# Funatiq/cuclark

Measured on AMD Instinct MI355X. Metric: Mreads/sec (10M x 150bp, k=31), higher is better.
Workload: dtype u64

## Files before the change

cuclark_amd/csrc/mic_engine.hip:

```cpp
#include "mi_clark.h"
#include "mic_internal.h"

#include <errno.h>
#include <stdarg.h>
#include <stdio.h>
#include <stdlib.h>
#include <string.h>
#include <time.h>

#include <sched.h>

#include <algorithm>
#include <mutex>
#include <string>
#include <atomic>
#include <thread>
#include <unistd.h>
#include <utility>
#include <vector>

static thread_local char g_err[512] = "";
thread_local uint64_t mic_build_reserved_hbm = 0;

namespace {
// ... 48 lines not shown
  if (!out) return MIC_E_INVALID;
  StreamPool& P = pool();
  std::lock_guard<std::mutex> lk(P.mu);
  out[0] = (uint32_t)P.all_streams.size(); out[1] = (uint32_t)P.free_streams.size();
  out[2] = (uint32_t)P.all_events.size(); out[3] = (uint32_t)P.free_events.size();
  return MIC_OK;
}

void mic_event_put(hipEvent_t ev) {
  if (!ev) return;
  (void)hipEventSynchronize(ev);
  StreamPool& P = pool();
  std::lock_guard<std::mutex> lk(P.mu);
  for (const auto& a : P.all_events) if (a.second == ev) { P.free_events.push_back(a); return; }
}
namespace {
std::mutex g_report_mu;
std::string g_report;
thread_local std::string t_report;

struct Batch {
  uint32_t* h_rp = nullptr; uint16_t* h_cont = nullptr;
  uint32_t* d_rp = nullptr; uint16_t* d_cont = nullptr;
  uint32_t* d_results = nullptr; uint32_t* d_rows = nullptr;
  uint32_t* d_flagged = nullptr; uint32_t* h_flagged = nullptr;
  uint32_t* d_peer = nullptr; uint32_t* d_acc = nullptr;
  uint32_t* d_crowd = nullptr;
  size_t first_read = 0, n_reads = 0, n_cont = 0, max_reads = 0, max_cont = 0;
  hipStream_t stream = nullptr;
  hipEvent_t done = nullptr, ev_up = nullptr, ev_k = nullptr;
  bool scheduled = false, resolved = true, extended = false;
};

}

struct mic_engine {
  mic_config cfg;
  int device = 0, n_cu = 256;
  hipStream_t stream = nullptr;
  hipStream_t up_stream = nullptr, down_stream = nullptr;
  bool db_loaded = false;
  uint4* slots = nullptr;
  uint4* side = nullptr;
  uint8_t* d_sizes = nullptr;
  MicTable table;
  int slot_class = 32;
  mic_db_info info;
  std::vector<Batch> batches;
  void* h_block = nullptr; void* d_block = nullptr;
  uint32_t* h_results = nullptr; uint32_t* h_rows = nullptr;
  size_t num_reads_total = 0;
  std::mutex submit_mu;
  uint32_t* d_flagged = nullptr; uint32_t flagged_cap = 0;
  uint32_t* d_crowd = nullptr; size_t crowd_reads = 0;
  hipEvent_t ev0 = nullptr, ev1 = nullptr;
  bool timed = false;
  size_t last_n_reads = 0;
  void* ingest = nullptr;
  uint32_t min_quality = 0;
  uint32_t low_complexity = 0;
  uint64_t reserve_hbm = 0;
  uint32_t part = 0, n_parts = 0;
  MicAbund abund;
  MicRollup rollup;
  MicDensity density;
  MicSplit split;
  MicKsketch ksketch;
  MicHitmap hitmap;
};

namespace {

const uint32_t kFlaggedCap = 1u << 16;

int set_device(const mic_engine* e) {
  MIC_TRY(hipSetDevice(e->device));
  return MIC_OK;
}

void fill_table(mic_engine* e, const MicBuildOut& b, uint64_t htsize, uint64_t s0, uint64_t s1, int key_bytes,
                uint32_t sampling, int layout, int m) {
  e->slots = b.slots;
  const bool parted = (layout == MIC_LAYOUT_SUPER || layout == MIC_LAYOUT_SUPER2) && (b.part_lo != 0 || b.part_hi != b.n_main);
  e->table.slots = parted ? b.slots - (ptrdiff_t)b.part_lo * 8 : b.slots;
  e->table.slot_lo = parted ? (uint32_t)b.part_lo : 0; e->table.slot_cnt = parted ? (uint32_t)(b.part_hi - b.part_lo) : 0;
  e->table.parted = parted ? 1 : 0;
  e->side = b.side;
  e->table.side = b.side; e->table.side_mask = b.side ? (uint32_t)(b.side_cells - 1) : 0;
  e->table.n_main = b.n_main;
  e->table.shard_start = s0;
  e->table.shard_end = s1;
  e->table.div = mic_make_div(htsize);
  e->table.k = e->cfg.k;
  e->table.layout = layout == MIC_LAYOUT_MINIMIZER ? 1 : (layout == MIC_LAYOUT_SUPER || layout == MIC_LAYOUT_SUPER2) ? 2 : 0;
  e->table.fwd = layout == MIC_LAYOUT_SUPER2 ? 1 : 0;
  e->table.m = m;
  e->table.sharded = (s0 != 0 || s1 != htsize) ? 1 : 0;
  e->table.sizes = e->d_sizes;
  mic_db_info& i = e->info;
  i.htsize = htsize; i.shard_start = s0; i.shard_end = s1;
  i.n_elems = b.n_elems; i.n_elems_file = b.n_elems_file;
  const uint64_t n_res = parted ? b.part_hi - b.part_lo : b.n_main;
  i.n_slots = n_res + b.n_overflow; i.n_overflow = b.n_overflow;
  i.part = e->n_parts > 1 ? e->part : 0; i.n_parts = e->n_parts > 1 ? e->n_parts : 0;
  i.part_slot_lo = parted ? b.part_lo : 0; i.part_slot_hi = parted ? b.part_hi : 0; i.n_slots_whole = b.n_main;
  i.side_kmers = b.side ? b.side_kmers : 0; i.side_bytes = b.side ? b.side_cells * 16 : 0;
// ... 400 lines not shown
  g_peer[from][to] = ok ? 1 : -1;
  return ok;
}
void mic_peer_enable_engines(mic_engine* const* engines, size_t n) {
  for (size_t i = 0; i < n; ++i)
    for (size_t j = 0; j < n; ++j)
      if (engines[i] && engines[j] && engines[i]->device != engines[j]->device) mic_peer_enable(engines[i]->device, engines[j]->device);
}

extern "C" {

const char* mic_last_error(void) { return g_err; }

int mic_device_count(int* count) {
  int n = 0;
  hipError_t e = hipGetDeviceCount(&n);
  if (e != hipSuccess) { *count = 0; return mic_set_error(MIC_E_NODEVICE, "hipGetDeviceCount: %s", hipGetErrorString(e)); }
  *count = n;
  return MIC_OK;
}

int mic_create(const mic_config* cfg, mic_engine** out) {
  if (!cfg || !out) return mic_set_error(MIC_E_INVALID, "null argument");
  if (cfg->k < 2 || cfg->k > 32) return mic_set_error(MIC_E_INVALID, "The k-mer length should be in [2,32].");
  if (cfg->num_targets > 65535) return mic_set_error(MIC_E_INVALID, "too many targets (%u > 65535)", cfg->num_targets);
  if (cfg->layout > MIC_LAYOUT_SUPER2) return mic_set_error(MIC_E_INVALID, "unknown table layout %u", cfg->layout);
  int n = 0;
  if (hipGetDeviceCount(&n) != hipSuccess || n == 0)
    return mic_set_error(MIC_E_NODEVICE, "no HIP device available: the MI355X engine cannot run (there is no CPU fallback)");
  int dev = cfg->device;
  if (dev < 0) { if (hipGetDevice(&dev) != hipSuccess) dev = 0; }
  if (dev >= n) return mic_set_error(MIC_E_INVALID, "device %d out of range (%d devices)", dev, n);
  hipDeviceProp_t prop;
  MIC_TRY(hipSetDevice(dev));
  MIC_TRY(hipGetDeviceProperties(&prop, dev));
  if (strncmp(prop.gcnArchName, "gfx950", 6) != 0)
    return mic_set_error(MIC_E_NODEVICE, "device %d is %s; this library carries gfx950 (MI355X) code objects only", dev, prop.gcnArchName);
  mic_engine* e = new (std::nothrow) mic_engine();
  if (!e) return mic_set_error(MIC_E_NOMEM, "out of host memory");
  e->cfg = *cfg;
  if (e->cfg.num_batches == 0) e->cfg.num_batches = 1;
  if (e->cfg.row_words == 0) e->cfg.row_words = 16;
  if (e->cfg.row_words < 2) e->cfg.row_words = 2;
  e->device = dev;
  e->n_cu = prop.multiProcessorCount;
  memset(&e->info, 0, sizeof(e->info));
  memset(&e->table, 0, sizeof(e->table));
  hipError_t he = mic_stream_get(&e->stream);
  if (he == hipSuccess) he = mic_stream_get(&e->up_stream);
  if (he == hipSuccess) he = mic_stream_get(&e->down_stream);
  if (he == hipSuccess) he = mic_event_get(&e->ev0, true);
  if (he == hipSuccess) he = mic_event_get(&e->ev1, true);
  if (he == hipSuccess) he = hipMalloc(&e->d_flagged, (size_t)(kFlaggedCap + 1) * 4);
  if (he != hipSuccess) { mic_destroy(e); return mic_set_error(MIC_E_HIP, "engine setup: %s", hipGetErrorString(he)); }
  e->flagged_cap = kFlaggedCap;
  *out = e;
  return MIC_OK;
}

int mic_destroy(mic_engine* e) {
  if (!e) return MIC_OK;
  hipSetDevice(e->device);
  hipDeviceSynchronize();
  mic_ingest_free(e);
  mic_gz_release(e);
  free_batches(e);
  if (e->slots) hipFree(e->slots);
  if (e->side) hipFree(e->side);
  if (e->d_sizes) hipFree(e->d_sizes);
  if (e->d_flagged) hipFree(e->d_flagged);
  if (e->d_crowd) hipFree(e->d_crowd);
  if (e->abund.d_counts) hipFree(e->abund.d_counts);
  if (e->rollup.d_counts) hipFree(e->rollup.d_counts);
  if (e->density.d_counts) hipFree(e->density.d_counts);
  if (e->ksketch.d_regs) hipFree(e->ksketch.d_regs);
  if (e->rollup.d_block) hipFree(e->rollup.d_block);
  if (e->ev0) mic_event_put(e->ev0);
  if (e->ev1) mic_event_put(e->ev1);
  if (e->stream) mic_stream_put(e->stream);
  if (e->up_stream) mic_stream_put(e->up_stream);
  if (e->down_stream) mic_stream_put(e->down_stream);
  delete e;
  return MIC_OK;
}

int mic_db_unload(mic_engine* e) {
  if (!e) return mic_set_error(MIC_E_INVALID, "null engine");
  int rc = set_device(e);
  if (rc) return rc;
  hipDeviceSynchronize();
  if (e->slots) hipFree(e->slots);
  if (e->side) hipFree(e->side);
  if (e->d_sizes) hipFree(e->d_sizes);
  e->slots = nullptr; e->side = nullptr; e->d_sizes = nullptr; e->db_loaded = false;
  memset(&e->info, 0, sizeof(e->info));
  return MIC_OK;
}

int mic_db_get_info(const mic_engine* e, mic_db_info* info) {
  if (!e || !info) return mic_set_error(MIC_E_INVALID, "null argument");
  if (!e->db_loaded) return mic_set_error(MIC_E_STATE, "no database loaded");
  *info = e->info;
  return MIC_OK;
}

int mic_debug_fetch_slots(mic_engine* e, uint64_t first, uint64_t n, uint32_t* out) {
  if (!e || !out) return mic_set_error(MIC_E_INVALID, "null argument");
  if (!e->db_loaded) return mic_set_error(MIC_E_STATE, "no database loaded");
  if (e->table.layout != 2 || e->table.parted) return mic_set_error(MIC_E_UNSUPPORTED, "slots are fetched from a whole super-k-mer table only");
  if (first > e->info.n_slots || n > e->info.n_slots - first) return mic_set_error(MIC_E_INVALID, "slots [%llu, +%llu) of %llu",
                                                                                   (unsigned long long)first, (unsigned long long)n, (unsigned long long)e->info.n_slots);
  int rc = set_device(e);
  if (rc) return rc;
  MIC_TRY(hipDeviceSynchronize());
  if (n) MIC_TRY(hipMemcpy(out, e->table.slots + first * 8, n * 128, hipMemcpyDeviceToHost));
  return MIC_OK;
}

const char* mic_db_last_build_report(void) {
  static thread_local std::string copy;
  std::lock_guard<std::mutex> lk(g_report_mu);
  copy = g_report;
  return copy.c_str();
// ... 572 lines not shown
  free(h_sz);
  for (Dev& dv : devs) {
    hipSetDevice(dv.device);
    if (dv.d_sz) hipFree(dv.d_sz);
    if (dv.d_ky) hipFree(dv.d_ky);
    if (dv.d_lb) hipFree(dv.d_lb);
  }
  return rc;
}

int mic_batch_check(mic_engine* e, size_t batch, int* done) {
  if (!e || batch >= e->batches.size() || !done) return mic_set_error(MIC_E_INVALID, "bad argument");
  Batch& B = e->batches[batch];
  if (!B.scheduled) { *done = 0; return MIC_OK; }
  hipError_t he = hipEventQuery(B.done);
  if (he == hipSuccess) *done = 1;
  else if (he == hipErrorNotReady) *done = 0;
  else return mic_set_error(MIC_E_HIP, "hipEventQuery: %s", hipGetErrorString(he));
  return MIC_OK;
}

int mic_thread_bind_near_device(mic_engine* e, int on) {
  if (!e) return mic_set_error(MIC_E_INVALID, "null engine");
  mic_bind_thread_near_device(e->device, on);
  return MIC_OK;
}

int mic_sync(mic_engine* e) {
  if (!e) return mic_set_error(MIC_E_INVALID, "null engine");
  int rc = set_device(e);
  if (rc) return rc;
  MIC_TRY(hipDeviceSynchronize());
  return MIC_OK;
}

int mic_batches_free(mic_engine* e) {
  if (!e) return mic_set_error(MIC_E_INVALID, "null engine");
  int rc = set_device(e);
  if (rc) return rc;
  hipDeviceSynchronize();
  free_batches(e);
  return MIC_OK;
}

int mic_query_device(mic_engine* e, const uint32_t* d_rp, const uint16_t* d_cont, size_t n_reads, uint32_t* d_results,
                     uint32_t* d_rows, void* stream) {
  if (!e || !d_rp || !d_cont || !d_results) return mic_set_error(MIC_E_INVALID, "null argument");
  if (!e->db_loaded) return mic_set_error(MIC_E_STATE, "no database loaded");
  if (n_reads > 0xFFFFFFF0ull) return mic_set_error(MIC_E_INVALID, "too many reads in one call");
  if (((uintptr_t)d_cont & 3) || ((uintptr_t)d_rp & 3)) return mic_set_error(MIC_E_INVALID, "d_containers and d_reads_pointer must be 4-byte aligned");
  int rc = set_device(e);
  if (rc) return rc;
  hipStream_t s = stream ? (hipStream_t)stream : e->stream;
  MIC_TRY(hipMemsetAsync(e->d_flagged, 0, 4, s));
  MicQueryArgs a;
  a.t = e->table; a.reads_ptr = d_rp; a.cont = d_cont; a.n_reads = (uint32_t)n_reads;
  a.row_words = e->cfg.row_words; a.results = d_results; a.rows = d_rows;
  a.flagged = e->d_flagged; a.flagged_cap = e->flagged_cap;
  if (e->table.side && n_reads > e->crowd_reads) {
    MIC_TRY(hipStreamSynchronize(s));
    if (e->d_crowd) { hipFree(e->d_crowd); e->d_crowd = nullptr; e->crowd_reads = 0; }
    MIC_TRY(hipMalloc(&e->d_crowd, mic_crowd_dims(n_reads).words * 4));
    e->crowd_reads = n_reads;
  }
  mic_crowd_attach(a, e->table.side ? e->d_crowd : nullptr, e->crowd_reads);
  MIC_TRY(hipEventRecord(e->ev0, s));
  MIC_TRY(mic_launch_query(a, e->slot_class, e->n_cu, s));
  MIC_TRY(hipEventRecord(e->ev1, s));
  e->timed = true;
  e->last_n_reads = n_reads;
  return MIC_OK;
}

int mic_last_query_ms(mic_engine* e, float* ms) {
  if (!e || !ms) return mic_set_error(MIC_E_INVALID, "null argument");
  if (!e->timed) return mic_set_error(MIC_E_STATE, "no query was launched");
  MIC_TRY(hipEventSynchronize(e->ev1));
  MIC_TRY(hipEventElapsedTime(ms, e->ev0, e->ev1));
  return MIC_OK;
}

int mic_last_crowd_stats(mic_engine* e, uint32_t out[4]) {
  if (!e || !out) return mic_set_error(MIC_E_INVALID, "null argument");
  out[0] = out[1] = out[2] = out[3] = 0;
  if (!e->timed || !e->d_crowd || !e->table.side) return MIC_OK;
  int rc = set_device(e);
  if (rc) return rc;
  MIC_TRY(hipEventSynchronize(e->ev1));
  MIC_TRY(hipMemcpy(out, e->d_crowd, 16, hipMemcpyDeviceToHost));
  return MIC_OK;
}

int mic_debug_fetch_crowd(mic_engine* e, uint32_t* out, size_t words, uint32_t caps[3]) {
  if (!e || !out || !caps) return mic_set_error(MIC_E_INVALID, "null argument");
  if (!e->d_crowd || !e->timed) return mic_set_error(MIC_E_STATE, "no work area");
  int rc = set_device(e);
  if (rc) return rc;
  const MicCrowdDims d = mic_crowd_dims(e->crowd_reads);
  caps[0] = d.pend_cap; caps[1] = d.item_cap; caps[2] = d.pool_cap;
  MIC_TRY(hipEventSynchronize(e->ev1));
  MIC_TRY(hipMemcpy(out, e->d_crowd, (words < d.words ? words : d.words) * 4, hipMemcpyDeviceToHost));
  return MIC_OK;
}

int mic_resolve_flagged_device(mic_engine* e, const uint32_t* d_rp, const uint16_t* d_cont, uint32_t* d_results,
                               uint32_t* d_rows, void* stream, size_t* n_resolved) {
  if (!e || !d_rp || !d_cont || !d_results) return mic_set_error(MIC_E_INVALID, "null argument");
  int rc = set_device(e);
  if (rc) return rc;
  hipStream_t s = stream ? (hipStream_t)stream : e->stream;
  uint32_t nf = 0;
  MIC_TRY(hipMemcpyAsync(&nf, e->d_flagged, 4, hipMemcpyDeviceToHost, s));
  MIC_TRY(hipStreamSynchronize(s));
  if (n_resolved) *n_resolved = nf;
  if (!nf) return MIC_OK;
  if (nf > e->flagged_cap) {
    if (n_resolved) *n_resolved = e->last_n_reads;
    return run_dense(e, d_rp, d_cont, nullptr, e->last_n_reads, d_results, d_rows, s);
  }
  return run_dense(e, d_rp, d_cont, e->d_flagged + 1, nf, d_results, d_rows, s);
}

int mic_merge_rows_device(mic_engine* e, const uint32_t* a, const uint32_t* b, uint32_t* out, size_t n, void* stream) {
  if (!e || !a || !b || !out) return mic_set_error(MIC_E_INVALID, "null argument");
  int rc = set_device(e);
  if (rc) return rc;
  MIC_TRY(mic_launch_merge_rows(a, b, out, e->cfg.row_words, n, nullptr, stream ? (hipStream_t)stream : e->stream));
  return MIC_OK;
}

int mic_result_from_rows_device(mic_engine* e, const uint32_t* rows, uint32_t* results, size_t n, void* stream) {
  if (!e || !rows || !results) return mic_set_error(MIC_E_INVALID, "null argument");
  int rc = set_device(e);
  if (rc) return rc;
  MIC_TRY(mic_launch_result_from_rows(rows, e->cfg.row_words, results, n, stream ? (hipStream_t)stream : e->stream));
  return MIC_OK;
}

int mic_result_from_dense_device(mic_engine* e, const uint32_t* d_counts, const uint32_t* d_ids, size_t n_ids, uint32_t* d_results,
                                 uint32_t* d_rows, void* stream) {
  if (!e || !d_counts || !d_results) return mic_set_error(MIC_E_INVALID, "null argument");
  int rc = set_device(e);
  if (rc) return rc;
  MIC_TRY(mic_launch_dense_finish(d_counts, d_ids, n_ids, e->cfg.num_targets ? e->cfg.num_targets : 1, d_results, d_rows,
                                 e->cfg.row_words, stream ? (hipStream_t)stream : e->stream));
  return MIC_OK;
}

int mic_probe_stats_device(mic_engine* e, const uint32_t* d_rp, const uint16_t* d_cont, size_t n_reads, uint64_t out[4]) {
  if (!e || !d_rp || !d_cont || !out) return mic_set_error(MIC_E_INVALID, "null argument");
  if (!e->db_loaded) return mic_set_error(MIC_E_STATE, "no database loaded");
  int rc = set_device(e);
  if (rc) return rc;
  unsigned long long* d = nullptr;
  unsigned long long h[4] = {0, 0, 0, 0};
  MIC_TRY(hipMalloc(&d, 32));
  hipError_t he = hipMemsetAsync(d, 0, 32, e->stream);
  if (he == hipSuccess) he = mic_launch_probe_stats(e->table, e->slot_class, d_rp, d_cont, n_reads, d, e->stream);
  if (he == hipSuccess) he = hipMemcpyAsync(h, d, 32, hipMemcpyDeviceToHost, e->stream);
  if (he == hipSuccess) he = hipStreamSynchronize(e->stream);
  hipFree(d);
  if (he != hipSuccess) return mic_set_error(MIC_E_HIP, "probe stats: %s", hipGetErrorString(he));
  for (int i = 0; i < 4; ++i) out[i] = h[i];
  return MIC_OK;
}

int mic_count_dense_device(mic_engine* e, const uint32_t* d_rp, const uint16_t* d_cont, const uint32_t* d_ids,
                           size_t n_ids, uint32_t* d_counts, void* stream) {
// ... 11 lines not shown
```

cuclark_amd/csrc/mic_kernels.hip:

```cpp
#include "mic_internal.h"
#include "mic_device.h"
#include "mic_ksketch.h"
#include "mic_hitmap.h"
#include "mic_join2.h"

#include <stdlib.h>
#include <type_traits>

#ifndef MIC_EXP
#define MIC_EXP 0
#endif
#ifndef MIC_FUNNEL64
#define MIC_FUNNEL64 1
#endif
#ifndef MIC_X
#define MIC_X 0
#endif
#if MIC_X & 8
__device__ unsigned long long g_entry_walk[3];
extern "C" int mic_debug_entry_walk(unsigned long long out[3], int reset) {
  if (hipMemcpyFromSymbol(out, HIP_SYMBOL(g_entry_walk), sizeof(g_entry_walk)) != hipSuccess) return -1;
  const unsigned long long z[3] = {0, 0, 0};
  if (reset && hipMemcpyToSymbol(HIP_SYMBOL(g_entry_walk), z, sizeof(z)) != hipSuccess) return -1;
  return 0;
}
#endif

namespace {

__device__ __forceinline__ uint4 load_slot_quarter(const uint4* p) {
  typedef unsigned int u4 __attribute__((ext_vector_type(4)));
  u4 t = __builtin_nontemporal_load((const u4*)p);
  return make_uint4(t.x, t.y, t.z, t.w);
}

__device__ __forceinline__ uint64_t kmer_from_dwords(uint32_t d0, uint32_t d1, uint32_t d2, int nt_in_dword, int k) {
  const int s = 2 * nt_in_dword;
  uint64_t a = ((uint64_t)d0 << 32) | d1;
#if MIC_FUNNEL64
  uint64_t x = (a << s) | ((uint64_t)d2 >> (32 - s));
#else
  uint64_t x = s ? ((a << s) | (uint64_t)(d2 >> (32 - s))) : a;
#endif
  return x >> (64 - 2 * k);
}


struct ReadAhead { uint32_t pp, pe, hdr, w; };

__device__ __forceinline__ void ahead_ptr(const MicQueryArgs& a, uint32_t r, ReadAhead& x) {
  if (r < a.n_reads) { x.pp = a.reads_ptr[r]; x.pe = a.reads_ptr[r + 1]; } else { x.pp = 0; x.pe = 0; }
}

__device__ __forceinline__ void ahead_window(const uint16_t* __restrict__ cont, uint32_t r, uint32_t n_reads, int lane,
                                             ReadAhead& x) {
  x.hdr = 0; x.w = 0;
  if (r < n_reads) {
    const uint32_t pp = __builtin_amdgcn_readfirstlane(x.pp);
    x.hdr = cont[pp];
    if (lane < 10) x.w = ((uint32_t)cont[pp + 1 + 2 * lane] << 16) | cont[pp + 2 + 2 * lane];
  }
}

__device__ __forceinline__ uint32_t window_word(const uint16_t* __restrict__ cont, uint32_t first, uint32_t cend,
                                                uint32_t base, int lane, bool use_ahead, const ReadAhead& x) {
  uint32_t w = 0;
  const uint32_t ci = first + base / 8 + 2 * lane;
  if (use_ahead) w = x.w;
  else if (lane < 10) w = ((ci < cend ? (uint32_t)cont[ci] : 0u) << 16) | (ci + 1 < cend ? (uint32_t)cont[ci + 1] : 0u);
  if (lane >= 10 || ci >= cend) w &= 0x0000FFFFu;
  if (lane >= 10 || ci + 1 >= cend) w &= 0xFFFF0000u;
  return w;
}

__device__ __forceinline__ uint32_t window_word_w(const uint16_t* __restrict__ cont, uint32_t first, uint32_t cend,
// ... 109 lines not shown
    m0 &= ~e0; m1 &= ~e1; m2 &= ~e2;
    row_add(acc, n_ent, overflow, l1, __popcll(e0) + __popcll(e1) + __popcll(e2), lane);
  }
}

template <typename ARGS>
__device__ __forceinline__ void finish_read(const RowAcc& acc, uint32_t n_ent, uint32_t total, uint32_t overflow,
                                            uint32_t r, const ARGS& a, int lane) {
  uint32_t bc = 0, bl = 0, sc = 0, sl = 0;
  uint32_t vbl = acc.label1, vbc = acc.count;
  if (n_ent > 1) {
    bl = __builtin_amdgcn_readlane(acc.label1, 0); bc = __builtin_amdgcn_readlane(acc.count, 0);
    for (uint32_t i = 1; i < n_ent; ++i) {
      const uint32_t l1 = __builtin_amdgcn_readlane(acc.label1, i);
      const uint32_t c = __builtin_amdgcn_readlane(acc.count, i);
      const bool over_best = c > bc || (c == bc && l1 < bl);
      const bool over_second = c > sc || (c == sc && l1 < sl);
      if (over_best) { sc = bc; sl = bl; bc = c; bl = l1; }
      else if (over_second) { sc = c; sl = l1; }
    }
    vbl = bl; vbc = bc;
  }
  uint32_t flags = 0;
  if (a.rows) {
    uint32_t* row = a.rows + (size_t)r * a.row_words;
    bool fits = n_ent <= a.row_words - 1 && !overflow;
    uint32_t rank = 0;
    for (uint32_t i = 0; i < n_ent; ++i) {
      uint32_t li = __builtin_amdgcn_readlane(acc.label1, i);
      rank += li < acc.label1;
    }
    bool big = (uint32_t)lane < n_ent && acc.count > 0xFFFF;
    if (__ballot(big)) fits = false;
    if (fits) {
      if ((uint32_t)lane < n_ent) row[1 + rank] = (acc.count << 16) | (acc.label1 - 1);
      if (lane == 0) row[0] = n_ent;
    } else {
      if (lane == 0) row[0] = MIC_ROW_INVALID;
      flags |= MIC_FLAG_ROW_OVERFLOW_;
    }
  }
  if (overflow) flags |= MIC_FLAG_ROW_OVERFLOW_;
  if (lane == 0 && !(MIC_X & 128)) {
    uint4 lo, hi;
    lo.x = total;
    lo.y = vbl;
    lo.z = vbc;
    lo.w = sl;
    hi.x = sc;
    hi.y = n_ent; hi.z = flags; hi.w = 0;
    uint4* out = (uint4*)(a.results + (size_t)r * 8);
    out[0] = lo; out[1] = hi;
  }
#if MIC_EXP & 2
  if (__builtin_expect(__builtin_amdgcn_readfirstlane(flags) != 0, 0)) if (a.flagged) {
#else
  if (__builtin_amdgcn_readfirstlane(flags) && a.flagged) {
#endif
    if (lane == 0) {
      uint32_t pos = atomicAdd(&a.flagged[0], 1u);
      if (pos < a.flagged_cap) a.flagged[1 + pos] = r;
    }
  }
}

template <bool KEY64>
__global__ void __launch_bounds__(256) query_kernel(const MicQueryArgs a) {
  const int lane = threadIdx.x & 63;
  const int j = lane & 3;
  const uint32_t wave0 = __builtin_amdgcn_readfirstlane(blockIdx.x * 4 + (threadIdx.x >> 6));
  const uint32_t n_waves = gridDim.x * 4;
  const MicTable& t = a.t;
  const int k = t.k;
  const uint4* __restrict__ slots = t.slots;
  const uint16_t* __restrict__ cont = a.cont;

  for (uint32_t r = wave0; r < a.n_reads; r += n_waves) {
    ReadAhead cur;
    ahead_ptr(a, r, cur);
    ahead_window(cont, r, a.n_reads, lane, cur);
    uint32_t pp = __builtin_amdgcn_readfirstlane(cur.pp);
    const uint32_t pe = __builtin_amdgcn_readfirstlane(cur.pe);
    RowAcc acc; acc.label1 = 0; acc.count = 0;
    uint32_t n_ent = 0, overflow = 0, total = 0;
    bool first_part = true;

    while (pp < pe) {
      const uint32_t plen = __builtin_amdgcn_readfirstlane(first_part ? cur.hdr : (uint32_t)cont[pp]);
      const bool ahead_ok = first_part;
      first_part = false;
      if (plen == 0) break;
      const uint32_t first = pp + 1;
      pp = first + (plen + 7) / 8;
      if (plen < (uint32_t)k) continue;
      const uint32_t nk = plen - k + 1;
      const uint32_t cend = pp;
      for (uint32_t base = 0; base < nk; base += 128) {
        const uint32_t w = window_word(cont, first, cend, base, lane, ahead_ok && base == 0, cur);
        Probe pr[2];
#pragma unroll
        for (int h = 0; h < 2; ++h) {
          const int idx = 4 * h + (lane >> 4);
          uint32_t d0 = bperm(idx, w), d1 = bperm(idx + 1, w), d2 = bperm(idx + 2, w);
          uint64_t kmer = kmer_from_dwords(d0, d1, d2, lane & 15, k);
          pr[h] = make_probe<KEY64>(t, kmer, base + 64 * h + lane < nk);
        }
        uint4 q[8]; uint32_t qlo[8], qhi[8]; uint32_t sl[8];
#pragma unroll
        for (int s = 0; s < 8; ++s) {
          const int src = 16 * (s & 3) + (lane >> 2);
          sl[s] = bperm(src, pr[s >> 2].slot);
// ... 682 lines not shown
                  }
                }
                more0 = same0 && !m0 && e0 < 5; more1 = same1 && !m1 && e1 < 5;
                e0 += more0 ? 1u : 0u; e1 += more1 ? 1u : 0u;
                if (!(__ballot(more0) | __ballot(more1))) break;
              }
              if (v0) { o0_ = hit0; y0_ = 0xFFFFFFFFu; }
              if (v1) { o1_ = hit1; y1_ = 0xFFFFFFFFu; }
              const bool n0 = v0 && !hit0 && (mz0 & MIC_S_NEXT), n1 = v1 && !hit1 && (mz1 & MIC_S_NEXT);
              if (__ballot(n0) | __ballot(n1)) {
                if (n0 && q0[5] <= t0) y0_ = q0[31];
                if (n1 && q1[5] <= t1) y1_ = q1[31];
              }
            }
          }
        };
        while (__ballot(sl0 != 0xFFFFFFFFu) | __ballot(sl1 != 0xFFFFFFFFu)) {
          uint32_t nx0, nx1;
          level(sl0, sl1, res0, res1, nx0, nx1);
          sl0 = nx0; sl1 = nx1;
        }
        tally2(res0, res1, acc, n_ent, overflow, total, lane);
      }
    }
    uint32_t t_hdr, t_pp, t_pe;
    asm volatile("s_waitcnt vmcnt(0)" ::: "memory");
    __builtin_amdgcn_wave_barrier();
    ahead_take(ahead_sel ? ahead1 : ahead0, n_pp, t_hdr, t_pp, t_pe);
    __builtin_amdgcn_wave_barrier();
    {
      uint64_t kp = (uint64_t)__builtin_amdgcn_kernarg_segment_ptr();
      asm volatile("" : "+s"(kp));
      const __attribute__((address_space(4))) MicQueryArgs* kc = (const __attribute__((address_space(4))) MicQueryArgs*)kp;
      struct { uint32_t* results; uint32_t* rows; uint32_t* flagged; uint32_t row_words, flagged_cap; } fa;
      fa.results = kc->results; fa.rows = kc->rows; fa.flagged = kc->flagged; fa.row_words = kc->row_words; fa.flagged_cap = kc->flagged_cap;
      finish_read(acc, n_ent, total, overflow, r, fa, lane);
    }
    ahead_issue(ahead_sel ? ahead0 : ahead1, t_pp, r + 3 * n_waves);
    ahead_sel ^= 1;
    cur_pp = n_pp; cur_pe = n_pe; cur_hdr = t_hdr; n_pp = t_pp; n_pe = t_pe;
  }
}


__device__ __forceinline__ uint64_t wballot(bool p) { return __builtin_amdgcn_ballot_w64(p); }
#if defined(__has_builtin) && __has_builtin(__builtin_amdgcn_writelane)
__device__ __forceinline__ int mic_writelane(int value, int lane, int old) { return __builtin_amdgcn_writelane(value, lane, old); }
#else
extern "C" __device__ int mic_writelane(int value, int lane, int old) __asm("llvm.amdgcn.writelane.i32");
#endif

static_assert(MIC_RMAX <= 32, "tally_counts sums the first two rows of lanes");
#define MIC_R_CROWDED (-16)
__device__ __forceinline__ void tally_counts(uint32_t lab1, uint32_t cnt, RowAcc& acc, uint32_t& n_ent, uint32_t& overflow,
                                             uint32_t& total, int lane) {
  uint64_t mm = wballot(lab1 != 0);
  while (mm) {
    const uint32_t l1 = __builtin_amdgcn_readlane(lab1, __builtin_ctzll(mm));
    const bool mine = lab1 == l1;
    mm &= ~wballot(mine);
    const uint32_t c = mine ? cnt : 0u;
    uint32_t sum = 0;
    {
      uint32_t v = c;
      v += (uint32_t)__builtin_amdgcn_update_dpp(0, (int)v, 0x111, 0xF, 0xF, true);
      v += (uint32_t)__builtin_amdgcn_update_dpp(0, (int)v, 0x112, 0xF, 0xF, true);
      v += (uint32_t)__builtin_amdgcn_update_dpp(0, (int)v, 0x114, 0xF, 0xF, true);
      v += (uint32_t)__builtin_amdgcn_update_dpp(0, (int)v, 0x118, 0xF, 0xF, true);
      sum = __builtin_amdgcn_readlane(v, 15) + __builtin_amdgcn_readlane(v, 31);
    }
    total += sum;
    if (wballot(acc.label1 == l1)) {
      if (acc.label1 == l1) acc.count += sum;
    } else if (n_ent < 64) {
      acc.label1 = (uint32_t)mic_writelane((int)l1, (int)n_ent, (int)acc.label1);
      acc.count = (uint32_t)mic_writelane((int)sum, (int)n_ent, (int)acc.count);
      ++n_ent;
    } else {
      overflow = 1;
    }
  }
}

template <int KK, int MM, bool FWD, bool PART>
__global__ void __launch_bounds__(64 * MIC_M_WPB, 32 / MIC_M_WPB) query_kernel_r(const MicQueryArgs a) {
  __shared__ uint4 s_stage[MIC_M_WPB][MIC_RMAX * MIC_MSTRIDE + (MIC_RMAX / 8 - 1) * MIC_R_SKEW];
  __shared__ uint16_t s_rec[MIC_M_WPB][132];
  __shared__ uint32_t s_ahead[MIC_M_WPB][2][64];
  __shared__ uint32_t s_part[PART ? MIC_M_WPB : 1][2];
  const int lane = threadIdx.x & 63;
  const int wv = __builtin_amdgcn_readfirstlane(threadIdx.x >> 6);
  uint4* stage = s_stage[wv];
  uint16_t* rec = s_rec[wv];
  const uint32_t wave0 = __builtin_amdgcn_readfirstlane(blockIdx.x * MIC_M_WPB + wv);
  const uint32_t n_waves = gridDim.x * MIC_M_WPB;
  const MicTable& t = a.t;
  if (PART) { if (lane == 0) { s_part[wv][0] = t.slot_lo; s_part[wv][1] = t.slot_cnt; } __builtin_amdgcn_wave_barrier(); }
  const int k = KK ? KK : t.k, m = MM ? MM : t.m, ctx = k - m;
  const uint4* __restrict__ slots = t.slots;
  const uint16_t* __restrict__ cont = a.cont;
  auto below = [](uint64_t mask) { return (uint32_t)__builtin_amdgcn_mbcnt_hi((uint32_t)(mask >> 32), __builtin_amdgcn_mbcnt_lo((uint32_t)mask, 0u)); };

  uint32_t* ahead0 = s_ahead[wv][0];
  uint32_t* ahead1 = s_ahead[wv][1];
  auto lane_copy = [&]() { int ln = lane; asm volatile("" : "+v"(ln)); return ln; };
  auto ahead_issue = [&](uint32_t* entry, uint32_t pp_w, uint32_t r_ptr, const int ln) {
    const uint64_t abase = ((uint64_t)(cont + pp_w)) & ~3ULL;
    const uint32_t rr = r_ptr < a.n_reads ? r_ptr : a.n_reads - 1;
    const uint64_t pbase = (uint64_t)(a.reads_ptr + rr) - 48;
    if (ln < 12)
      __builtin_amdgcn_global_load_lds((const __attribute__((address_space(1))) void*)((const uint32_t*)abase + lane),
                                       (__attribute__((address_space(3))) void*)entry, 4, 0, 0);
    uint64_t pb = pbase + 48;
    asm volatile("" : "+s"(pb));
    if (ln < 2)
      __builtin_amdgcn_global_load_lds((const __attribute__((address_space(1))) void*)((const uint32_t*)pb + lane),
                                       (__attribute__((address_space(3))) void*)(entry + 12), 4, 0, 0);
  };
  auto ahead_take = [&](const uint32_t* entry, uint32_t pp_w, uint32_t& hdr, uint32_t& npp, uint32_t& npe) {
    const uint32_t raw = entry[lane];
    npp = __builtin_amdgcn_readlane(raw, 12); npe = __builtin_amdgcn_readlane(raw, 13);
    const bool odd = (((uint64_t)(cont + pp_w)) >> 1) & 1;
    const uint32_t first = __builtin_amdgcn_readfirstlane(raw);
    hdr = odd ? first >> 16 : first & 0xFFFFu;
  };
  auto ahead_word = [&](const uint32_t* entry, uint32_t pp_w) {
    const uint32_t raw = entry[lane];
    const bool odd = (((uint64_t)(cont + pp_w)) >> 1) & 1;
    const uint32_t up = (uint32_t)__builtin_amdgcn_update_dpp(0, (int)raw, 0x101, 0xF, 0xF, true);
    return __builtin_amdgcn_perm(up, raw, odd ? 0x05040706u : 0x03020504u);
  };
  uint32_t cur_pp, cur_pe, cur_hdr, n_pp, n_pe, ahead_sel;
  {
// ... 103 lines not shown
                   W2 = (uint32_t)__builtin_amdgcn_ds_bpermute(a0 + 8, (int)wd), W3 = (uint32_t)__builtin_amdgcn_ds_bpermute(a0 + 12, (int)wd);
    uint32_t G0 = __builtin_amdgcn_alignbit(W0, W1, tsh), G1 = __builtin_amdgcn_alignbit(W1, W2, tsh), G2 = __builtin_amdgcn_alignbit(W2, W3, tsh);
    uint32_t key, xhi;
    region_x(G0, G1, key, xhi);
    bool rev = false;
    if (!FWD) {
      const uint32_t sh = 96u - 2u * (uint32_t)(k + ctx);
      const uint32_t r0 = __builtin_bitreverse32(G2), r1 = __builtin_bitreverse32(G1), r2 = __builtin_bitreverse32(G0);
      uint32_t q0, q1, q2;
      if (KK != 0 && sh != 0) {
        q0 = swap_comp_pairs(__builtin_amdgcn_alignbit(r0, r1, 33u - sh), __builtin_amdgcn_alignbit(r0, r1, 31u - sh));
        q1 = swap_comp_pairs(__builtin_amdgcn_alignbit(r1, r2, 33u - sh), __builtin_amdgcn_alignbit(r1, r2, 31u - sh));
        q2 = swap_comp_pairs(r2 << (sh - 1u), r2 << (sh + 1u));
      } else {
        q0 = sh ? __builtin_amdgcn_alignbit(r0, r1, 32u - sh) : r0;
        q1 = sh ? __builtin_amdgcn_alignbit(r1, r2, 32u - sh) : r1;
        q2 = r2 << sh;
        q0 = swap_comp_pairs(q0 >> 1, q0 << 1); q1 = swap_comp_pairs(q1 >> 1, q1 << 1); q2 = swap_comp_pairs(q2 >> 1, q2 << 1);
      }
      uint32_t kr, hr;
      region_x(q0, q1, kr, hr);
      rev = hr < xhi || (hr == xhi && kr < key);
      G0 = rev ? q0 : G0; G1 = rev ? q1 : G1; G2 = rev ? q2 : G2;
      key = rev ? kr : key; xhi = rev ? hr : xhi;
    }
    const int jmaxf = qa - i0, jminf = jmaxf - n + 1;
    const int jmax = rev ? ctx - jminf : jmaxf, jmin = rev ? ctx - jmaxf : jminf;
    uint32_t cur = vr ? sslot_of_x32(key, xhi, (uint32_t)t.n_main) : 0xFFFFFFFFu;
    bool mine = vr;
    if (PART) {
      mine = vr && cur - s_part[wv][0] < s_part[wv][1];
      cur = mine ? cur : 0xFFFFFFFFu;
    }
    L.G0 = G0; L.G1 = G1; L.G2 = G2; L.cur = cur;
    L.jmax = jmax; L.jmin = jmin; L.remaining = mine ? n : 0;
  };
  auto issue = [&](const uint32_t cur, const uint32_t nrun, const int ln) __attribute__((always_inline)) {
    uint32_t sidx[MIC_RMAX / 8];
    __builtin_amdgcn_wave_barrier();
    if (ln < MIC_RMAX) ((uint32_t*)stage)[lane] = cur;
    __builtin_amdgcn_wave_barrier();
    uint32_t so = (uint32_t)(uintptr_t)(__attribute__((address_space(3))) void*)stage;
    asm volatile("" : "+s"(so));
#pragma unroll
    for (int i = 0; i < MIC_RMAX / 8; ++i) sidx[i] = ((const uint32_t*)stage)[8 * i + (lane >> 3)];
#pragma unroll
    for (int i = 0; i < MIC_RMAX / 8; ++i) {
      if (8u * i >= nrun) break;
      if (sidx[i] != 0xFFFFFFFFu)
        __builtin_amdgcn_global_load_lds((const __attribute__((address_space(1))) void*)(slots + (uint64_t)sidx[i] * 8 + (lane & 7)),
                                         (__attribute__((address_space(3))) void*)(uintptr_t)(so + 16u * (64 + MIC_R_SKEW) * (uint32_t)i), 16, 0, 0);
    }
  };
  auto consume = [&](Round& L, RowAcc& acc, uint32_t& n_ent, uint32_t& overflow, uint32_t& total, uint32_t& cg) __attribute__((always_inline)) {
    const uint32_t G0 = L.G0, G1 = L.G1, G2 = L.G2;
    uint32_t key, xhi_;
    region_x(G0, G1, key, xhi_);
    const int jmax = L.jmax, jmin = L.jmin;
    uint32_t cur = L.cur;
    int remaining = L.remaining;
    for (;;) {
      asm volatile("s_waitcnt vmcnt(0)" ::: "memory");
      __builtin_amdgcn_wave_barrier();
      const bool vl = cur != 0xFFFFFFFFu;
      const uint32_t* q = (const uint32_t*)(stage + (vl ? staged_at((uint32_t)lane) : 0));
      const uint4 ka = *(const uint4*)q;
      const uint2 kb = *(const uint2*)(q + 4);
      uint32_t e = (ka.x < key) + (ka.y < key) + (ka.z < key) + (ka.w < key) + (kb.x < key) + (kb.y < key);
      const uint32_t mz = q[30];
      const uint64_t m_vl = wballot(vl);
      uint64_t m_more = m_vl & wballot(e < 6), m_pos = 0;
      e = e < 5 ? e : 5;
#if MIC_X & 8
      uint32_t ew_pass = 0;
#endif
      for (;;) {
        uint32_t e3 = e + (e << 1);
        asm volatile("" : "+v"(e3));
        uint32_t g = q[e], g1 = q[e + 1], S0 = q[6 + e3], S1 = q[7 + e3], S2 = q[8 + e3], pl = q[24 + e];
        asm volatile("" : "+v"(S2));
        const uint64_t m_same = m_more & wballot(g == key);
        const uint64_t m_next = wballot(g1 == key);
        const uint32_t d0 = G0 ^ S0, d1 = G1 ^ S1, d2 = G2 ^ S2;
        const uint64_t m_hit = m_same & (k > 16
                                             ? wballot(((d0 & ((1u << ((32 - 2 * ctx) & 31)) - 1u)) | (d1 >> xsh)) == 0)
                                             : wballot((((((uint64_t)d0 << 32) | d1) << (2 * ctx)) >> (64 - 2 * m)) == 0));
        const uint32_t dl = d0 >> (32 - 2 * ctx);
        const uint32_t dr = k > 16 ? __builtin_amdgcn_alignbit(d1, d2, xsh)
                                        : (uint32_t)((((((uint64_t)d0 << 32) | d1)) << ((2 * k) & 63)) >> 32);
        const int left = __builtin_ctz(dl | (1u << (2 * ctx))) >> 1;
        const int right = __builtin_clz(dr | (1u << (31 - 2 * ctx))) >> 1;
        const int hi = left < jmax ? left : jmax, lo = ctx - right > jmin ? ctx - right : jmin;
        const uint32_t range = ((2u << (hi & 31)) - 1u) & (~0u << (lo & 31));
        const uint32_t hits = __builtin_amdgcn_inverse_ballot_w64(m_hit) ? (uint32_t)__popc((pl >> 16) & range) : 0u;
#if MIC_X & 8
        const bool ew_hit = wballot(hits != 0) != 0;
        if (lane == 0 && ew_pass < 2u) atomicAdd(&g_entry_walk[ew_pass], 1ull);
        if (lane == 0 && ew_pass == 1u && ew_hit) atomicAdd(&g_entry_walk[2], 1ull);
        ++ew_pass;
#endif
        const uint32_t lab_new = (pl & 0xFFFFu) + 1u;
#if !(MIC_X & 16)
        tally_counts(hits ? lab_new : 0u, hits, acc, n_ent, overflow, total, lane);
#endif
#if MIC_X & 32
        break;
#endif
#if !(MIC_X & 1)
        remaining = __builtin_amdgcn_inverse_ballot_w64(m_hit & wballot(pl < 0x10000u)) ? MIC_R_CROWDED : remaining;
#endif
        remaining -= (int)hits;
        m_pos = wballot(remaining > 0);
        m_more = m_same & m_pos & wballot(e < 5);
#if !(MIC_X & 256)
        m_more &= m_next;
#endif
        e += __builtin_amdgcn_inverse_ballot_w64(m_more) ? 1u : 0u;
        if (!m_more) break;
      }
#if MIC_X & 64
      break;
#endif
      const uint64_t m_nx = m_pos & wballot((mz & MIC_S_NEXT) != 0);
      if (!m_nx) break;
      cur = 0xFFFFFFFFu;
      if (__builtin_amdgcn_inverse_ballot_w64(m_nx) && q[5] <= key) cur = q[31];
      if (!wballot(cur != 0xFFFFFFFFu)) break;
      remaining = (cur == 0xFFFFFFFFu && remaining > 0) ? 0 : remaining;
      issue(cur, MIC_RMAX, lane_copy());
    }
    if (!(MIC_X & 2) && __builtin_expect(wballot(remaining <= MIC_R_CROWDED) != 0, 0)) {
      const bool crowded = remaining <= MIC_R_CROWDED;
      const uint32_t n_c = (uint32_t)__popcll(wballot(crowded));
      uint64_t kpv = (uint64_t)__builtin_amdgcn_kernarg_segment_ptr();
      asm volatile("" : "+v"(kpv));
      const MicQueryArgs* kv = (const MicQueryArgs*)kpv;
      uint32_t* cw = kv->crowd;
      uint32_t* itb = kv->crowd_items;
      const uint32_t icap = kv->crowd_item_cap;
      uint32_t ib = 0xFFFFFFFFu;
      if (cw != nullptr && cg != MIC_CG_DENSE) {
        uint32_t v = 0;
        if (lane == 0) v = atomicAdd(&cw[1], n_c);
        ib = __builtin_amdgcn_readfirstlane(v);
      }
      asm volatile("" : "+v"(ib));
      const bool room = ib <= icap && n_c <= icap - ib;
      if (crowded && room) {
        uint32_t* it = itb + 8 * ((size_t)ib + below(wballot(crowded)));
        it[0] = G0; it[1] = G1; it[2] = G2; it[3] = (uint32_t)jmin | ((uint32_t)jmax << 8);
        it[4] = cg;
      }
      cg = __builtin_amdgcn_readfirstlane(room ? (ib | ((n_c - 1u) << 27)) : MIC_CG_DENSE);
    }
  };
  auto finish = [&](const RowAcc& acc, uint32_t n_ent, uint32_t total, uint32_t overflow, uint32_t r, const uint32_t cg) __attribute__((always_inline)) {
    uint32_t spilled = 0;
    if (!(MIC_X & 4) && __builtin_expect(cg != MIC_CG_NONE, 0)) {
      uint64_t kpv = (uint64_t)__builtin_amdgcn_kernarg_segment_ptr();
      asm volatile("" : "+v"(kpv));
      const MicQueryArgs* kv = (const MicQueryArgs*)kpv;
      uint32_t* cw = kv->crowd;
      uint32_t* pool = kv->crowd_pool;
      const uint32_t pcap = kv->crowd_pend_cap, wcap = kv->crowd_pool_cap;
      uint32_t p = 0xFFFFFFFFu, off = 0;
      if (cg != MIC_CG_DENSE) {
        if (lane == 0) { p = atomicAdd(&cw[0], 1u); off = atomicAdd(&cw[2], 2u * n_ent); }
        p = __builtin_amdgcn_readfirstlane(p); off = __builtin_amdgcn_readfirstlane(off);
      }
      asm volatile("" : "+v"(p), "+v"(off));
      const bool room = off <= wcap && 2u * n_ent <= wcap - off;
      if (p < pcap) {
        uint32_t* pd = cw + MIC_CROWD_HDR + 8 * (size_t)p;
        if (lane == 0) { pd[0] = r; pd[1] = total; pd[2] = room ? (n_ent | (overflow << 8)) : 0xFFFFFFFFu; pd[3] = off; pd[4] = cg; }
        if (room && (uint32_t)lane < n_ent) { uint32_t* pe_ = pool + (size_t)off + 2 * lane; pe_[0] = acc.label1; pe_[1] = acc.count; }
      }
      spilled = __builtin_amdgcn_readfirstlane((p < pcap && room) ? 1u : 0u);
      if (!spilled) {
        if (lane == 0 && cw != nullptr && cg != MIC_CG_DENSE) atomicAdd(&cw[3], 1u);
        overflow = 1;
      }
    }
    if (!spilled) {
      uint64_t kp = (uint64_t)__builtin_amdgcn_kernarg_segment_ptr();
      asm volatile("" : "+s"(kp));
      const __attribute__((address_space(4))) MicQueryArgs* kc = (const __attribute__((address_space(4))) MicQueryArgs*)kp;
      struct { uint32_t* results; uint32_t* rows; uint32_t* flagged; uint32_t row_words, flagged_cap; } fa;
      fa.results = kc->results; fa.rows = kc->rows; fa.flagged = kc->flagged; fa.row_words = kc->row_words; fa.flagged_cap = kc->flagged_cap;
      finish_read(acc, n_ent, total, overflow, r, fa, lane);
    }
  };

  uint32_t r = wave0; bool p_valid = false;
  auto step = [&](Round& P, Round& N) __attribute__((always_inline)) -> bool {
    const bool have = r < a.n_reads;
    uint32_t pp = cur_pp;
    const uint32_t pe = cur_pe;
    bool shape = false, simple = false;
    uint32_t n_nrun = 0, plen0 = 0, pp1 = 0;
    uint32_t slot2 = J2_NONE;
    if (have) {
      plen0 = cur_hdr; pp1 = pp + 1 + (plen0 + 7) / 8;
      shape = plen0 - (uint32_t)k < 128u && pp1 == pe;
      if (!shape && plen0 - (uint32_t)k < 128u && pp1 < pe) {
        const uint32_t rel = pp1 - cur_pp + (uint32_t)((((uint64_t)(cont + cur_pp)) >> 1) & 1);
        if (rel < 24u) {
          const uint32_t v = (ahead_sel ? ahead0 : ahead1)[rel >> 1];
          slot2 = __builtin_amdgcn_readfirstlane((rel & 1u) ? v >> 16 : v & 0xFFFFu);
          shape = slot2 == 0;
        }
      }
      uint32_t n_wd = 0, R = MIC_RMAX + 1u, g0 = 0xFFFFFFFFu;
      if (PIPE && shape) {
        R = front(pp + 1, pp1, 0u, plen0 - (uint32_t)k + 1u, true, n_wd, NoGap{});
      } else if constexpr (PIPE) {
        const uint32_t odd = (uint32_t)((((uint64_t)(cont + cur_pp)) >> 1) & 1);
        const uint32_t* entry = ahead_sel ? ahead0 : ahead1;
        const J2Shape j2 = j2_shape(plen0, slot2, pe - pp, odd, (uint32_t)k,
                                    [&](uint32_t u) { return (uint32_t)__builtin_amdgcn_readfirstlane(j2_half(entry[u >> 1], u)); });
        if (__builtin_expect(j2.ok != 0u, 0)) {
          R = front(pp + 1, pp1, 0u, j2.n_act, true, n_wd, Gap{j2.len1, j2.b2, j2.g0});
          g0 = j2.g0;
        }
      }
      if (PIPE && R <= MIC_RMAX) { setup(n_wd, 0u, R, N, n_nrun, Gap{0u, 0u, g0}); simple = true; }
    }
    if (PIPE && p_valid) {
      RowAcc acc; acc.label1 = 0; acc.count = 0;
      uint32_t n_ent = 0, overflow = 0, total = 0, cg = MIC_CG_NONE;
      consume(P, acc, n_ent, overflow, total, cg);
      finish(acc, n_ent, total, overflow, r - n_waves, cg);
    } else {
      asm volatile("s_waitcnt vmcnt(0)" ::: "memory");
    }
    if (!have) return false;
    if (!simple) {
      RowAcc acc; acc.label1 = 0; acc.count = 0;
      uint32_t n_ent = 0, overflow = 0, total = 0, cg = MIC_CG_NONE;
      auto chunk = [&](const uint32_t first, const uint32_t cend, const uint32_t base, const uint32_t nk, const bool use_ahead) __attribute__((always_inline)) {
        uint32_t wd;
        const uint32_t R = front(first, cend, base, nk, use_ahead, wd, NoGap{});
        for (uint32_t rbase = 0; rbase < R; rbase += MIC_RMAX) {
          Round L; uint32_t nrun;
          setup(wd, rbase, R, L, nrun, NoGap{});
          issue(L.cur, nrun, lane_copy());
          consume(L, acc, n_ent, overflow, total, cg);
        }
      };
      if (!PIPE && shape) chunk(pp + 1, pp1, 0u, plen0 - (uint32_t)k + 1u, true);
      else {
        bool first_part = true;
        while (pp < pe) {
          uint32_t plen;
          {
            const uint32_t rel = pp - cur_pp + (uint32_t)((((uint64_t)(cont + cur_pp)) >> 1) & 1);
            if (first_part) plen = cur_hdr;
            else if (rel < 24u) {
              const uint32_t v = (ahead_sel ? ahead0 : ahead1)[rel >> 1];
              plen = __builtin_amdgcn_readfirstlane((rel & 1u) ? v >> 16 : v & 0xFFFFu);
            } else plen = __builtin_amdgcn_readfirstlane((uint32_t)cont[pp]);
          }
          const bool ahead_ok = first_part;
          first_part = false;
          if (plen == 0) break;
          const uint32_t first = pp + 1;
          pp = first + (plen + 7) / 8;
          if (plen < (uint32_t)k) continue;
          const uint32_t nk = plen - k + 1;
          const uint32_t cend = pp;
          for (uint32_t base = 0; base < nk; base += 128) chunk(first, cend, base, nk, ahead_ok && base == 0);
        }
      }
      finish(acc, n_ent, total, overflow, r, cg);
    }
    uint32_t t_hdr, t_pp, t_pe;
    __builtin_amdgcn_wave_barrier();
    ahead_take(ahead_sel ? ahead1 : ahead0, n_pp, t_hdr, t_pp, t_pe);
    __builtin_amdgcn_wave_barrier();
    const int ln = lane_copy();
    ahead_issue(ahead_sel ? ahead0 : ahead1, t_pp, r + 3 * n_waves, ln);
    ahead_sel ^= 1;
    cur_pp = n_pp; cur_pe = n_pe; cur_hdr = t_hdr; n_pp = t_pp; n_pe = t_pe;
    p_valid = simple;
    if (simple) issue(N.cur, n_nrun, ln);
    r += n_waves;
    return true;
  };
  Round Ra, Rb;
  while (step(Ra, Rb) && step(Rb, Ra)) {}
}

__global__ void __launch_bounds__(256) crowd_finish_kernel(const MicQueryArgs a) {
  const int lane = threadIdx.x & 63;
  const uint32_t wave0 = __builtin_amdgcn_readfirstlane(blockIdx.x * 4 + (threadIdx.x >> 6)), n_waves = gridDim.x * 4;
  const uint32_t* __restrict__ cw = a.crowd;
  const uint32_t pcap = a.crowd_pend_cap;
  uint32_t np = cw[0];
  np = np < pcap ? np : pcap;
  const uint32_t* __restrict__ pend = cw + MIC_CROWD_HDR;
  const uint32_t* __restrict__ items = a.crowd_items;
  const uint32_t* __restrict__ pool = a.crowd_pool;
  const uint4* __restrict__ side = a.t.side;
  const uint32_t smask = a.t.side_mask;
  const int k = a.t.k, ctx = k - a.t.m;
  for (uint32_t p = wave0; p < np; p += n_waves) {
    const uint4 h = *(const uint4*)(pend + 8 * (size_t)p);
    const uint32_t r = __builtin_amdgcn_readfirstlane(h.x), meta = __builtin_amdgcn_readfirstlane(h.z), off = __builtin_amdgcn_readfirstlane(h.w);
    uint32_t total = __builtin_amdgcn_readfirstlane(h.y);
    uint32_t g = __builtin_amdgcn_readfirstlane(pend[8 * (size_t)p + 4]);
    if (meta == 0xFFFFFFFFu) continue;
    uint32_t n_ent = meta & 0xFFu, overflow = (meta >> 8) & 1u;
    RowAcc acc; acc.label1 = 0; acc.count = 0;
    if ((uint32_t)lane < n_ent) { const uint2 e = *(const uint2*)(pool + off + 2 * lane); acc.label1 = e.x; acc.count = e.y; }
    while (g != MIC_CG_NONE) {
      const uint32_t ib = g & 0x7FFFFFFu, n_c = (g >> 27) + 1u;
      g = __builtin_amdgcn_readfirstlane(items[8 * (size_t)ib + 4]);
      for (uint32_t b = 0; b < n_c; b += 4) {
        const uint32_t idx = b + ((uint32_t)lane >> 4);
        const bool valid = idx < n_c;
        uint4 it = make_uint4(0, 0, 0, 0);
        if (valid) it = *(const uint4*)(items + 8 * (size_t)(ib + idx));
        const int jmin = (int)(it.w & 0xFFu), jmax = (int)((it.w >> 8) & 0xFFu);
        int j = jmin + (lane & 15);
        bool go = valid && j <= jmax;
        j = go ? j : jmin;
        const uint64_t K = s_extract(it.x, it.y, it.z, ctx - j, k);
// ... 568 lines not shown
```

Before: 2386.

## Skip redundant flagged-counter memset and specialize finish path for uncrowded rows

The host now copies the flagged count into pinned memory and remembers when it was zero, so the next query on the same stream skips the memset that resets the counter. In the kernel, consume returns whether any lane was crowded. The pipelined path then calls a finish variant that statically drops the spill branch when no lane was crowded. tally_counts ballots on nonzero counts instead of masking labels, with the reduction split into helpers and a few branch hints added; the debug counters also change, which risks stale-state bugs if the counter is touched elsewhere.

Result: no change. 2397 (median of 2 runs) (+0.5%).

```diff
diff --git a/cuclark_amd/csrc/mic_engine.hip b/cuclark_amd/csrc/mic_engine.hip
--- a/cuclark_amd/csrc/mic_engine.hip
+++ b/cuclark_amd/csrc/mic_engine.hip
@@ -124,6 +124,7 @@
   size_t num_reads_total = 0;
   std::mutex submit_mu;
   uint32_t* d_flagged = nullptr; uint32_t flagged_cap = 0;
+  uint32_t* h_flagged_n = nullptr; bool flagged_zero = false; hipStream_t flagged_stream = nullptr;
   uint32_t* d_crowd = nullptr; size_t crowd_reads = 0;
   hipEvent_t ev0 = nullptr, ev1 = nullptr;
   bool timed = false;
@@ -630,6 +631,7 @@
   if (he == hipSuccess) he = mic_event_get(&e->ev0, true);
   if (he == hipSuccess) he = mic_event_get(&e->ev1, true);
   if (he == hipSuccess) he = hipMalloc(&e->d_flagged, (size_t)(kFlaggedCap + 1) * 4);
+  if (he == hipSuccess) he = hipHostMalloc((void**)&e->h_flagged_n, 64, hipHostMallocDefault);
   if (he != hipSuccess) { mic_destroy(e); return mic_set_error(MIC_E_HIP, "engine setup: %s", hipGetErrorString(he)); }
   e->flagged_cap = kFlaggedCap;
   *out = e;
@@ -647,6 +649,7 @@
   if (e->side) hipFree(e->side);
   if (e->d_sizes) hipFree(e->d_sizes);
   if (e->d_flagged) hipFree(e->d_flagged);
+  if (e->h_flagged_n) hipHostFree(e->h_flagged_n);
   if (e->d_crowd) hipFree(e->d_crowd);
   if (e->abund.d_counts) hipFree(e->abund.d_counts);
   if (e->rollup.d_counts) hipFree(e->rollup.d_counts);
@@ -1325,7 +1328,9 @@
   int rc = set_device(e);
   if (rc) return rc;
   hipStream_t s = stream ? (hipStream_t)stream : e->stream;
-  MIC_TRY(hipMemsetAsync(e->d_flagged, 0, 4, s));
+  const bool counter_is_zero = e->flagged_zero;
+  e->flagged_zero = false; e->flagged_stream = s;
+  if (!counter_is_zero) MIC_TRY(hipMemsetAsync(e->d_flagged, 0, 4, s));
   MicQueryArgs a;
   a.t = e->table; a.reads_ptr = d_rp; a.cont = d_cont; a.n_reads = (uint32_t)n_reads;
   a.row_words = e->cfg.row_words; a.results = d_results; a.rows = d_rows;
@@ -1382,11 +1387,14 @@
   int rc = set_device(e);
   if (rc) return rc;
   hipStream_t s = stream ? (hipStream_t)stream : e->stream;
-  uint32_t nf = 0;
-  MIC_TRY(hipMemcpyAsync(&nf, e->d_flagged, 4, hipMemcpyDeviceToHost, s));
+  MIC_TRY(hipMemcpyAsync(e->h_flagged_n, e->d_flagged, 4, hipMemcpyDeviceToHost, s));
   MIC_TRY(hipStreamSynchronize(s));
+  const uint32_t nf = *(volatile uint32_t*)e->h_flagged_n;
   if (n_resolved) *n_resolved = nf;
-  if (!nf) return MIC_OK;
+  if (!nf) {
+    if (e->timed && s == e->flagged_stream) e->flagged_zero = true;
+    return MIC_OK;
+  }
   if (nf > e->flagged_cap) {
     if (n_resolved) *n_resolved = e->last_n_reads;
     return run_dense(e, d_rp, d_cont, nullptr, e->last_n_reads, d_results, d_rows, s);
diff --git a/cuclark_amd/csrc/mic_kernels.hip b/cuclark_amd/csrc/mic_kernels.hip
--- a/cuclark_amd/csrc/mic_kernels.hip
+++ b/cuclark_amd/csrc/mic_kernels.hip
@@ -7,9 +7,6 @@
 #include <stdlib.h>
 #include <type_traits>
 
-#ifndef MIC_EXP
-#define MIC_EXP 0
-#endif
 #ifndef MIC_FUNNEL64
 #define MIC_FUNNEL64 1
 #endif
@@ -17,10 +14,10 @@
 #define MIC_X 0
 #endif
 #if MIC_X & 8
-__device__ unsigned long long g_entry_walk[3];
-extern "C" int mic_debug_entry_walk(unsigned long long out[3], int reset) {
+__device__ unsigned long long g_entry_walk[6];
+extern "C" int mic_debug_entry_walk(unsigned long long out[6], int reset) {
   if (hipMemcpyFromSymbol(out, HIP_SYMBOL(g_entry_walk), sizeof(g_entry_walk)) != hipSuccess) return -1;
-  const unsigned long long z[3] = {0, 0, 0};
+  const unsigned long long z[6] = {0, 0, 0, 0, 0, 0};
   if (reset && hipMemcpyToSymbol(HIP_SYMBOL(g_entry_walk), z, sizeof(z)) != hipSuccess) return -1;
   return 0;
 }
@@ -236,11 +233,7 @@
     uint4* out = (uint4*)(a.results + (size_t)r * 8);
     out[0] = lo; out[1] = hi;
   }
-#if MIC_EXP & 2
   if (__builtin_expect(__builtin_amdgcn_readfirstlane(flags) != 0, 0)) if (a.flagged) {
-#else
-  if (__builtin_amdgcn_readfirstlane(flags) && a.flagged) {
-#endif
     if (lane == 0) {
       uint32_t pos = atomicAdd(&a.flagged[0], 1u);
       if (pos < a.flagged_cap) a.flagged[1 + pos] = r;
@@ -1029,33 +1022,36 @@
 
 static_assert(MIC_RMAX <= 32, "tally_counts sums the first two rows of lanes");
 #define MIC_R_CROWDED (-16)
+__device__ __forceinline__ uint32_t sum_run_lanes(uint32_t v) {
+  v += (uint32_t)__builtin_amdgcn_update_dpp(0, (int)v, 0x111, 0xF, 0xF, true);
+  v += (uint32_t)__builtin_amdgcn_update_dpp(0, (int)v, 0x112, 0xF, 0xF, true);
+  v += (uint32_t)__builtin_amdgcn_update_dpp(0, (int)v, 0x114, 0xF, 0xF, true);
+  v += (uint32_t)__builtin_amdgcn_update_dpp(0, (int)v, 0x118, 0xF, 0xF, true);
+  return __builtin_amdgcn_readlane(v, 15) + __builtin_amdgcn_readlane(v, 31);
+}
+
+__device__ __forceinline__ void tally_row(RowAcc& acc, uint32_t& n_ent, uint32_t& overflow, uint32_t l1, uint32_t sum) {
+  if (wballot(acc.label1 == l1)) {
+    if (acc.label1 == l1) acc.count += sum;
+  } else if (n_ent < 64) {
+    acc.label1 = (uint32_t)mic_writelane((int)l1, (int)n_ent, (int)acc.label1);
+    acc.count = (uint32_t)mic_writelane((int)sum, (int)n_ent, (int)acc.count);
+    ++n_ent;
+  } else {
+    overflow = 1;
+  }
+}
+
 __device__ __forceinline__ void tally_counts(uint32_t lab1, uint32_t cnt, RowAcc& acc, uint32_t& n_ent, uint32_t& overflow,
                                              uint32_t& total, int lane) {
-  uint64_t mm = wballot(lab1 != 0);
+  uint64_t mm = wballot(cnt != 0);
   while (mm) {
     const uint32_t l1 = __builtin_amdgcn_readlane(lab1, __builtin_ctzll(mm));
     const bool mine = lab1 == l1;
     mm &= ~wballot(mine);
-    const uint32_t c = mine ? cnt : 0u;
-    uint32_t sum = 0;
-    {
-      uint32_t v = c;
-      v += (uint32_t)__builtin_amdgcn_update_dpp(0, (int)v, 0x111, 0xF, 0xF, true);
-      v += (uint32_t)__builtin_amdgcn_update_dpp(0, (int)v, 0x112, 0xF, 0xF, true);
-      v += (uint32_t)__builtin_amdgcn_update_dpp(0, (int)v, 0x114, 0xF, 0xF, true);
-      v += (uint32_t)__builtin_amdgcn_update_dpp(0, (int)v, 0x118, 0xF, 0xF, true);
-      sum = __builtin_amdgcn_readlane(v, 15) + __builtin_amdgcn_readlane(v, 31);
-    }
+    const uint32_t sum = sum_run_lanes(mine ? cnt : 0u);
     total += sum;
-    if (wballot(acc.label1 == l1)) {
-      if (acc.label1 == l1) acc.count += sum;
-    } else if (n_ent < 64) {
-      acc.label1 = (uint32_t)mic_writelane((int)l1, (int)n_ent, (int)acc.label1);
-      acc.count = (uint32_t)mic_writelane((int)sum, (int)n_ent, (int)acc.count);
-      ++n_ent;
-    } else {
-      overflow = 1;
-    }
+    tally_row(acc, n_ent, overflow, l1, sum);
   }
 }
 
@@ -1265,7 +1261,7 @@
                                          (__attribute__((address_space(3))) void*)(uintptr_t)(so + 16u * (64 + MIC_R_SKEW) * (uint32_t)i), 16, 0, 0);
     }
   };
-  auto consume = [&](Round& L, RowAcc& acc, uint32_t& n_ent, uint32_t& overflow, uint32_t& total, uint32_t& cg) __attribute__((always_inline)) {
+  auto consume = [&](Round& L, RowAcc& acc, uint32_t& n_ent, uint32_t& overflow, uint32_t& total, uint32_t& cg) __attribute__((always_inline)) -> bool {
     const uint32_t G0 = L.G0, G1 = L.G1, G2 = L.G2;
     uint32_t key, xhi_;
     region_x(G0, G1, key, xhi_);
@@ -1308,13 +1304,13 @@
         const uint32_t hits = __builtin_amdgcn_inverse_ballot_w64(m_hit) ? (uint32_t)__popc((pl >> 16) & range) : 0u;
 #if MIC_X & 8
         const bool ew_hit = wballot(hits != 0) != 0;
-        if (lane == 0 && ew_pass < 2u) atomicAdd(&g_entry_walk[ew_pass], 1ull);
-        if (lane == 0 && ew_pass == 1u && ew_hit) atomicAdd(&g_entry_walk[2], 1ull);
+        if (lane == 0) atomicAdd(&g_entry_walk[ew_pass < 3u ? ew_pass : 3u], 1ull);
+        if (lane == 0 && ew_hit) atomicAdd(&g_entry_walk[ew_pass ? 4 : 5], 1ull);
         ++ew_pass;
 #endif
         const uint32_t lab_new = (pl & 0xFFFFu) + 1u;
 #if !(MIC_X & 16)
-        tally_counts(hits ? lab_new : 0u, hits, acc, n_ent, overflow, total, lane);
+        tally_counts(lab_new, hits, acc, n_ent, overflow, total, lane);
 #endif
 #if MIC_X & 32
         break;
@@ -1335,14 +1331,15 @@
       break;
 #endif
       const uint64_t m_nx = m_pos & wballot((mz & MIC_S_NEXT) != 0);
-      if (!m_nx) break;
+      if (__builtin_expect(m_nx == 0, 1)) break;
       cur = 0xFFFFFFFFu;
       if (__builtin_amdgcn_inverse_ballot_w64(m_nx) && q[5] <= key) cur = q[31];
       if (!wballot(cur != 0xFFFFFFFFu)) break;
       remaining = (cur == 0xFFFFFFFFu && remaining > 0) ? 0 : remaining;
       issue(cur, MIC_RMAX, lane_copy());
     }
-    if (!(MIC_X & 2) && __builtin_expect(wballot(remaining <= MIC_R_CROWDED) != 0, 0)) {
+    const bool any_crowded = !(MIC_X & 2) && wballot(remaining <= MIC_R_CROWDED) != 0;
+    if (__builtin_expect(any_crowded, 0)) {
       const bool crowded = remaining <= MIC_R_CROWDED;
       const uint32_t n_c = (uint32_t)__popcll(wballot(crowded));
       uint64_t kpv = (uint64_t)__builtin_amdgcn_kernarg_segment_ptr();
@@ -1366,10 +1363,11 @@
       }
       cg = __builtin_amdgcn_readfirstlane(room ? (ib | ((n_c - 1u) << 27)) : MIC_CG_DENSE);
     }
+    return any_crowded;
   };
-  auto finish = [&](const RowAcc& acc, uint32_t n_ent, uint32_t total, uint32_t overflow, uint32_t r, const uint32_t cg) __attribute__((always_inline)) {
+  auto finish = [&](const RowAcc& acc, uint32_t n_ent, uint32_t total, uint32_t overflow, uint32_t r, const uint32_t cg, const bool may_spill) __attribute__((always_inline)) {
     uint32_t spilled = 0;
-    if (!(MIC_X & 4) && __builtin_expect(cg != MIC_CG_NONE, 0)) {
+    if (!(MIC_X & 4) && may_spill && __builtin_expect(cg != MIC_CG_NONE, 0)) {
       uint64_t kpv = (uint64_t)__builtin_amdgcn_kernarg_segment_ptr();
       asm volatile("" : "+v"(kpv));
       const MicQueryArgs* kv = (const MicQueryArgs*)kpv;
@@ -1441,8 +1439,8 @@
     if (PIPE && p_valid) {
       RowAcc acc; acc.label1 = 0; acc.count = 0;
       uint32_t n_ent = 0, overflow = 0, total = 0, cg = MIC_CG_NONE;
-      consume(P, acc, n_ent, overflow, total, cg);
-      finish(acc, n_ent, total, overflow, r - n_waves, cg);
+      if (__builtin_expect(consume(P, acc, n_ent, overflow, total, cg), 0)) finish(acc, n_ent, total, overflow, r - n_waves, cg, true);
+      else finish(acc, n_ent, total, overflow, r - n_waves, MIC_CG_NONE, false);
     } else {
       asm volatile("s_waitcnt vmcnt(0)" ::: "memory");
     }
@@ -1484,7 +1482,7 @@
           for (uint32_t base = 0; base < nk; base += 128) chunk(first, cend, base, nk, ahead_ok && base == 0);
         }
       }
-      finish(acc, n_ent, total, overflow, r, cg);
+      finish(acc, n_ent, total, overflow, r, cg, true);
     }
     uint32_t t_hdr, t_pp, t_pe;
     __builtin_amdgcn_wave_barrier();
```
